# batra-mlp-lab/visdial

Measured on AMD Instinct MI355X. Metric: QA-rounds/sec training mn-att-ques-im-hist+disc (batch 20x10x100), higher is better.
Workload: dtype f32 operands and results; the option recurrence multiplies the EXACT 3-way bf16 split of both operands (9 bf16 MFMA products per fp32 product, f32 accumulate: fp32-grade, errors at the f32 MFMA's own level) -- its two step kernels and its weight-gradient contraction; f32 MFMA (v_mfma_f32_32x32x2_f32

## Files before the change

### visdial_amd/csrc/comm.hip

```cpp
#include <dlfcn.h>

#include "common.h"
#include "rt_core.h"
#include "../../include/visdial_hip.h"

namespace {

struct NcclUniqueId { char internal[128]; };
typedef void* NcclComm;
typedef int NcclResult;
enum { kNcclFloat32 = 7, kNcclSum = 0 };

struct Rccl {
  void* lib = nullptr;
  NcclResult (*GetUniqueId)(NcclUniqueId*) = nullptr;
  NcclResult (*CommInitRank)(NcclComm*, int, NcclUniqueId, int) = nullptr;
  NcclResult (*CommDestroy)(NcclComm) = nullptr;
  NcclResult (*AllReduce)(const void*, void*, size_t, int, int, NcclComm, hipStream_t) = nullptr;
  NcclResult (*GroupStart)() = nullptr;
  NcclResult (*GroupEnd)() = nullptr;
  const char* (*GetErrorString)(NcclResult) = nullptr;
  NcclResult (*GetVersion)(int*) = nullptr;
};

// ... 152 lines not shown
  if (g.stream) (void)hipStreamSynchronize(g.stream);
  NcclResult r = g.api.CommDestroy(g.comm);
  release_local();
  if (r != 0) {
    vd_set_error("vd_comm_destroy: ncclCommDestroy -> %s", g.api.GetErrorString(r));
    return VD_ERR_HIP;
  }
  return VD_OK;
}

int vd_model_allreduce_grads(vd_model* m) {
  VdRange r("vd_model_allreduce_grads");
  VD_CHECK_ARG(m, "vd_model_allreduce_grads: null model");
  VD_CHECK_ARG(g.comm, "vd_model_allreduce_grads: no communicator (vd_comm_init first)");
  VD_CHECK_ARG(m->cur >= 0, "vd_model_allreduce_grads: no backward pass has been enqueued");
  int dev = -1;
  VD_HIP(hipGetDevice(&dev));
  VD_CHECK_ARG(dev == g.device, "vd_model_allreduce_grads: communicator lives on device %d, current device is %d", g.device, dev);
  int64_t lo = 0, hi = 0;
  int rc = vd_model_encoder_range(m, &lo, &hi);
  if (rc != VD_OK) return rc;
  const bool split = hi > lo && m->enc_grads_recorded;
  if (split) {
    VD_HIP(hipStreamWaitEvent(g.stream, m->ev_enc_grads, 0));
    VD_NCCL(g.api.AllReduce(m->G + lo, m->G + lo, (size_t)(hi - lo), kNcclFloat32, kNcclSum, g.comm, g.stream));
    VD_HIP(hipEventRecord(g.ev_b1, g.stream));
    VD_HIP(hipEventRecord(g.ev_tail_t, m->s_main));
  }
  g.timed = split;
  VD_HIP(hipEventRecord(g.ev_tail, m->s_main));
// ... 26 lines not shown
```

### visdial_amd/csrc/rt_core.h

```cpp
#pragma once
#include <math.h>
#include <stdarg.h>
#include <stdlib.h>
#include <string.h>

#include <algorithm>
#include <map>
#include <memory>
#include <numeric>
#include <random>
#include <string>
#include <vector>

#include "../../include/visdial_hip.h"
#include "common.h"
#include "paths.h"

int vd_lstm2_forward_p(const vd_lstm2_fwd_t* st, int nstacks, int H, int flags, hipStream_t stream);
int vd_lstm2_backward_p(const vd_lstm2_bwd_t* st, int nstacks, int H, int flags, hipStream_t stream);

int vd_img_drop_gather(const float* pre, const uint8_t* mask1, float* xdrop, int N, int R, int S2, int H, float scale, hipStream_t stream);
int vd_img_common_forward_p(const float* pre, const uint8_t* mask1, const float* xdrop, const float* Wc, const float* bc, const float* qc,
                            const uint8_t* mask2, float* iqc, int N, int R, int S2, int H, int Kc, float scale, int flags, hipStream_t stream);
int vd_img_tr_backward_p(const float* dz, const float* Wc, const float* p, const float* datt, const uint8_t* mask1, float* dpre, int N, int R,
// ... 150 lines not shown
  vd_model_params p;
  int flags = 0;
  std::string enc_name, dec_name;
  std::vector<vdrt::Tensor> spec;
  std::map<std::string, int> index;
  long numel = 0;
  float *W = nullptr, *G = nullptr, *M = nullptr, *V = nullptr;
  std::map<std::string, vdrt::DevBuf> ws;
  std::map<std::string, vdrt::DevBuf> ext_masks;
  hipStream_t s_main = nullptr, s_side = nullptr;
  hipStream_t s_wg = nullptr;
  bool wg_active = false, wg_used = false;
  std::vector<hipEvent_t> ev_pool;
  size_t ev_next = 0;
  hipEvent_t ev_enc_grads = nullptr;
  hipEvent_t ev_updated = nullptr;
  bool updated_recorded = false;
  bool enc_grads_recorded = false;
  hipEvent_t ev_loss = nullptr, ev_prof[6] = {nullptr, nullptr, nullptr, nullptr, nullptr, nullptr};
  bool training = true, streams = true, prof_valid = false;
  long step = 0;
  int adam_t = 0;
  double lr = 1e-3;
  vdrt::BatchSlot slot[2];
  int cur = -1, uploaded = -1;
  float* loss_host = nullptr;
  long loss_cap = 0, loss_n = 0;
  bool loss_is_sum = false;
  std::unique_ptr<vdrt::Encoder> enc;
  std::unique_ptr<vdrt::Decoder> dec;
// ... 70 lines not shown
  VD_HIP(hipEventRecord(e, from));
  VD_HIP(hipStreamWaitEvent(side, e, 0));
  return VD_OK;
}
inline int join_stream(vd_model* m, hipStream_t side, hipStream_t to) { return fork_stream(m, side, to); }
inline hipStream_t side_stream(vd_model* m, hipStream_t cur) { return m->streams ? m->s_side : cur; }
inline int wg_fork(vd_model* m, hipStream_t cur, hipStream_t* out) {
  *out = cur;
  if (!m->wg_active || !m->s_wg) return VD_OK;
  VD_TRY(fork_stream(m, cur, m->s_wg));
  m->wg_used = true;
  *out = m->s_wg;
  return VD_OK;
}

inline int drop_mask(vd_model* m, const std::string& site, size_t numel, float p, hipStream_t s, uint8_t** out) {
  *out = nullptr;
  if (!m->training || p <= 0.f) return VD_OK;
  auto it = m->ext_masks.find(site);
  if (it != m->ext_masks.end()) {
    VD_CHECK_ARG(it->second.bytes >= numel, "dropout mask '%s' holds %zu bytes, the batch needs %zu", site.c_str(),
                 it->second.bytes, numel);
    *out = static_cast<uint8_t*>(it->second.p);
    return VD_OK;
  }
  if (!m->ext_masks.empty()) {
    vd_set_error("external dropout masks are set but none for site '%s'", site.c_str());
    return VD_ERR_STATE;
  }
  uint8_t* buf = nullptr;
// ... 46 lines not shown
    x = x_; M = M_; tanh_ = tanh;
    VD_TRY(ws_get(m, name + ".y", (size_t)M * out, &y));
    VD_TRY(vd_gemm_nt(x, in, Wp(m, name + ".W"), in, Wp(m, name + ".b"), y, out, (int)M, (int)out, (int)in,
                      tanh ? VD_ACT_TANH : VD_ACT_NONE, 0, s));
    if (y_out) *y_out = y;
    return VD_OK;
  }
  int backward(vd_model* m, hipStream_t s, const float* dy, bool need_dx, float** dx_out) {
    const float* d = dy;
    if (tanh_) {
      float* dpre;
      VD_TRY(ws_get(m, name + ".dpre", (size_t)M * out, &dpre));
      VD_TRY(vd_tanh_backward(dy, y, dpre, M * out, s));
      d = dpre;
    }
    VD_TRY(vd_gemm_tn_acc(d, out, x, in, Gp(m, name + ".W"), in, (int)out, (int)in, (int)M, 0, s));
    VD_TRY(vd_colsum_acc(d, out, (int)M, (int)out, Gp(m, name + ".b"), s));
    if (dx_out) *dx_out = nullptr;
    if (need_dx) {
      float* dx;
      VD_TRY(ws_get(m, name + ".dx", (size_t)M * in, &dx));
      VD_TRY(vd_gemm_nn(d, out, Wp(m, name + ".W"), in, nullptr, dx, in, (int)M, (int)in, (int)out, 0, s));
      if (dx_out) *dx_out = dx;
    }
    return VD_OK;
  }
};

struct CatLinear {
  std::string name;
  std::vector<long> dims;
  long D = 0, H = 0, N = 0;
// ... 122 lines not shown
      } else {
        VD_TRY(vd_gemm_nn(x, D, Wx(m), 4 * H, Wp(m, name + ".b"), gates, 4 * H, T * N, (int)(4 * H), (int)D, 0, s));
      }
      VD_TRY(vd_lstm_forward(gates, (int64_t)N * 4 * H, 4 * H, nullptr, mask, Wh(m), h0, c0, gates_out, h, c, T, N, (int)H, flags, s));
    }
    if (h_out) *h_out = h;
    return VD_OK;
  }
  int param_grads(vd_model* m, hipStream_t s, const std::vector<bool>& need_dx, std::vector<float*>* dxs) {
    const long TN = (long)T * N;
    float* dW = Gp(m, name + ".W");
    float* dWh = dW + D * 4 * H;
    const bool by_rows = rows && rows->act;
    auto dense_fits = [&](long Mrows, long K) { return vd_tn_kmajor_fits(Mrows, 4 * H, K); };
    auto wg_flags = [&](long Mrows) { return (m->flags & VD_FLAG_BF16) && vd_tn_split_tiles(Mrows, 4 * H) ? VD_FLAG_BF16 : 0; };
    if (by_rows && !(T > 1 && dense_fits(H, (long)(T - 1) * N))) {
      if (rows->n_act1 > 0)
        VD_TRY(vd_gemm_tn_rows_acc(h, H, rows->prev1, gates, 4 * H, rows->act1, dWh, 4 * H, (int)H, (int)(4 * H), rows->n_act1, s));
    } else if (T > 1) {
      VD_TRY(vd_gemm_tn_acc(h, H, gates + (long)N * 4 * H, 4 * H, dWh, 4 * H, (int)H, (int)(4 * H), (T - 1) * N, wg_flags(H), s));
    }
    if (h0) VD_TRY(vd_gemm_tn_acc(h0, H, gates, 4 * H, dWh, 4 * H, (int)H, (int)(4 * H), N, 0, s));
    VD_TRY(vd_colsum_acc(gates, 4 * H, (int)TN, (int)(4 * H), Gp(m, name + ".b"), s));
    if (dxs) dxs->assign(parts.size(), nullptr);
    long roff = 0;
    for (size_t i = 0; i < parts.size(); ++i) {
      if (by_rows && !dense_fits(parts[i], TN)) {
        if (rows->n_act > 0)
          VD_TRY(vd_gemm_tn_rows_acc(xs[i], parts[i], rows->act, gates, 4 * H, rows->act, dW + roff * 4 * H, 4 * H, (int)parts[i],
                                     (int)(4 * H), rows->n_act, s));
      } else {
        VD_TRY(vd_gemm_tn_acc(xs[i], parts[i], gates, 4 * H, dW + roff * 4 * H, 4 * H, (int)parts[i], (int)(4 * H), (int)TN, wg_flags(parts[i]), s));
      }
      if (need_dx.empty() || need_dx[i]) {
        float* dx;
        VD_TRY(ws_get(m, name + ".dx" + std::to_string(i), (size_t)TN * parts[i], &dx));
        VD_TRY(vd_gemm_nt(gates, 4 * H, Wx(m) + roff * 4 * H, 4 * H, nullptr, dx, parts[i], (int)TN, (int)parts[i], (int)(4 * H),
                          VD_ACT_NONE, 0, s));
        if (dxs) (*dxs)[i] = dx;
      }
      roff += parts[i];
    }
    return VD_OK;
  }
  int backward(vd_model* m, hipStream_t s, const float* dh_seq, const float* dh_last, const std::vector<bool>& need_dx,
               std::vector<float*>* dxs) {
    if (gradPrevOutput) {
// ... 42 lines not shown
```

### visdial_amd/csrc/rt_decoders.h

```cpp
#pragma once
#include "rt_encoders.h"

namespace vdrt {

int option_cache_resolve(vd_model* m, BatchSlot& sl, const int32_t* options, long NO, int To, hipStream_t s);

struct Decoder {
  virtual ~Decoder() {}
  virtual void declare(vd_model* m) = 0;
  virtual int forward_backward(vd_model* m, BatchSlot& b, bool only_forward) = 0;
  virtual int retrieve(vd_model* m, BatchSlot& b) = 0;
  virtual int retrieve_lhood(vd_model*, BatchSlot&) {
    vd_set_error("vd_model_retrieve_lhood: the live-row log-likelihood head scores candidates of decoder 'gen'; this model's decoder is 'disc'");
    return VD_ERR_ARG;
  }
  virtual int gen_begin(vd_model*, const int32_t*, int) { return no_gen(); }
  virtual int gen_step(vd_model*, const int32_t*, float*) { return no_gen(); }
  virtual int gen_select(vd_model*, const int32_t*, int) { return no_gen(); }
  virtual int gen_beam_search(vd_model*, int, int, int, int, int32_t*, double*) { return no_gen(); }
  virtual int gen_sample(vd_model*, int, int, int, double, const double*, int32_t*, double*) { return no_gen(); }
  static int no_gen() {
    vd_set_error("sampling / beam search only for the generative decoder (model.lua:436-438)");
    return VD_ERR_STATE;
  }
// ... 89 lines not shown
      VD_TRY(vd_memset(d_optH, 0, (long)NO * H * 4, s));
      VD_TRY(vd_embed_scatter_acc(d_optH, b.opt_uid, nullptr, d_optH_full, NOfull, (int)H, 1.f, s));
    }
    VD_TRY(stage_loss(m, loss_rows, N, false, s));
    m->scores = scores;
    m->prof_valid = !only_forward;
    if (only_forward) return VD_OK;
    VD_TRY(fork_stream(m, s, sd));
    float *dc, *dtab;
    int32_t* perm = b.opt_sort_perm;
    VD_TRY(ws_get(m, "opt.dc", (size_t)NO * H, &dc));
    VD_TRY(ws_get(m, "opt.dtable", (size_t)(V + 1) * 4 * H, &dtab));
    VD_CHECK_ARG(perm, "decoder 'disc': the batch slot carries no option-token sort");
    VD_TRY(vd_memset(dtab, 0, (V + 1) * 4 * H * 4, sd));
    VD_HIP(hipEventRecord(m->ev_prof[2], s));
    m->wg_active = m->streams && m->s_wg && (flags & VD_FLAG_BF16) != 0;
    m->wg_used = false;
    auto enc_bwd = [&]() -> int {
      VdRange r("encoder backward");
      VD_TRY(m->enc->backward(m, sd, b, d_enc));
      VD_PROBE_REC(1, sd);
      if (m->wg_used) VD_PROBE_REC(2, m->s_wg);
      if (m->wg_used) {
        VD_TRY(fork_stream(m, sd, m->s_wg));
        VD_HIP(hipEventRecord(m->ev_enc_grads, m->s_wg));
      } else {
        VD_HIP(hipEventRecord(m->ev_enc_grads, sd));
      }
      m->enc_grads_recorded = true;
      return VD_OK;
    };
    {
      VdRange r("disc: option LSTM backward");
      if (c16) VD_TRY(vd_lstm_backward_c16(Wopt + E * 4 * H, gates16, c, d_optH, dc, To, NO, (int)H, s));
      else VD_TRY(vd_lstm_backward(Wopt + E * 4 * H, gates, c, nullptr, nullptr, d_optH, nullptr, dc, nullptr, nullptr, nullptr, To, NO, (int)H, flags, s));
    }
    VD_HIP(hipEventRecord(m->ev_prof[3], s));
    VD_TRY(enc_bwd());
// ... 634 lines not shown
```

### visdial_amd/csrc/rt_encoders.h

```cpp
#pragma once
#include "rt_core.h"

namespace vdrt {

struct Encoder {
  virtual ~Encoder() {}
  virtual void declare(vd_model* m) = 0;
  virtual int forward(vd_model* m, hipStream_t s, BatchSlot& b, float** out) = 0;
  virtual int backward(vd_model* m, hipStream_t s, BatchSlot& b, const float* grad_out) = 0;
  virtual std::vector<SeqLSTM>* rnnLayers() { return nullptr; }
  virtual int seqLen(const BatchSlot& b) const { return b.q.T; }
};

inline int tick_flags(const vd_model* m) { return m->flags & VD_FLAG_BF16; }

inline int causal_mask(vd_model* m, int B, int R, uint8_t** out) {
  const std::string key = "causal." + std::to_string(B);
  DevBuf& d = m->ws[key];
  const size_t n = (size_t)B * R * R;
  if (!d.p) {
    std::vector<uint8_t> host(n);
    for (int r = 0; r < B * R; ++r)
      for (int j = 0; j < R; ++j) host[(size_t)r * R + j] = j > (r % R) ? 1 : 0;
    VD_HIP(hipMalloc(&d.p, n + 16));
// ... 288 lines not shown
    const float* dcur;
    VD_TRY(dropout_fwd(m, "att.du1", du1d, m_u, 2.f, (long)N * H, s, &dcur));
    float *dpre, *dscore;
    VD_TRY(ws_get(m, "att.dpre", (size_t)b.B * S2 * H, &dpre));
    VD_TRY(ws_get(m, "att.dscore", (size_t)N * S2, &dscore));
    VD_TRY(vd_memset(dpre, 0, (long)b.B * S2 * H * 4, s));
    for (int i = L - 1; i >= 0; --i) {
      const std::string sf = hop_sfx(i);
      float *dqc, *duq, *dun;
      VD_TRY(ws_get(m, "att.dqc" + sf, (size_t)N * K, &dqc));
      VD_TRY(ws_get(m, "att.du0" + sf, (size_t)N * H, &dun));
      VD_TRY(vd_img_att_backward(iqc[i], Wp(m, "att" + sf + ".W"), pre, m1, m2[i], patt[i], dcur, Gp(m, "att" + sf + ".W"),
                                 Gp(m, "att" + sf + ".b"), dqc, dscore, N, R, S2, (int)H, (int)K, sc, s));
      hipStream_t sw;
      VD_TRY(wg_fork(m, s, &sw));
      VD_TRY(vd_colsum_acc(iqc[i], K, N * S2, (int)K, Gp(m, "img_common" + sf + ".b"), sw));
      VD_TRY(vd_img_common_wgrad_p(iqc[i], pre, m1, xdrop, Gp(m, "img_common" + sf + ".W"), N, R, S2, (int)H, (int)K, sc, iflags, sw));
      VD_TRY(vd_img_tr_backward_p(iqc[i], Wp(m, "img_common" + sf + ".W"), patt[i], dcur, m1, dpre, N, R, S2, (int)H, (int)K, sc, iflags, sw));
      VD_TRY(ques_common[i].backward(m, s, dqc, true, &duq));
      VD_TRY(vd_axpby(duq, dcur, dun, (long)N * H, 1.f, 1.f, s));
      dcur = dun;
    }
    hipStream_t sw;
    VD_TRY(wg_fork(m, s, &sw));
    VD_TRY(img_proj.backward(m, sw, dpre, false, nullptr));
    *du0 = const_cast<float*>(dcur);
    return VD_OK;
  }
};

struct GraphEncoder : Encoder {
  bool memory_ = false, san_ = false, qi_ = false, qh_ = false;
  TextBranches text;
  MemoryBlock memory;
  SANBlock san;
  CatLinear qi, qh;
  explicit GraphEncoder(const std::string& name) {
    memory_ = name.rfind("mn", 0) == 0;
    san_ = name.find("att") != std::string::npos;
    qi_ = name == "mn-ques-im-hist";
// ... 347 lines not shown
```

### visdial_amd/csrc/runtime.hip

```cpp
#include <errno.h>
#include <float.h>

#include "rt_decoders.h"

using namespace vdrt;

vd_model::~vd_model() {}

namespace {

int upload_tokens(BatchSlot& sl, SeqTok& ss, const std::string& tag, const int32_t* rows_major, int N, int T, bool sorted, hipStream_t s) {
  ss.T = T;
  ss.N = N;
  ss.present = true;
  ss.sorted = sorted;
  const size_t TN = (size_t)T * N;
  const size_t total = sorted ? 7 * TN + 2 * (size_t)N + T : TN;
  int32_t* stage = nullptr;
  VD_TRY(pin_get(sl.pinned, tag + ".stage", total * sizeof(int32_t), (void**)&stage));
  int32_t* tok = stage;
  std::vector<int> len(sorted ? N : 0);
  for (int n = 0; n < N; ++n) {
    int first = T;
    for (int t = 0; t < T; ++t) {
// ... 203 lines not shown
  sl.tree_ok = false;
  const long V = m->p.vocabSize;
  for (size_t r = 0; r < (size_t)N * O; ++r) {
    bool run = true;
    for (int t = 0; t < T; ++t) {
      const int32_t a = oin[r * T + t], b = oout[r * T + t];
      if (a < 0 || a > V || b < 0 || b > V || (a != 0 && !run)) return VD_OK;
      run = run && a != 0;
    }
  }
  VD_TRY(tree_chunks(m, sl, oin, oout, N, O, T, 0, O, s));
  sl.tree_ok = true;
  return VD_OK;
}

extern "C" {

int vd_model_create(const vd_model_params* p, const char* encoder, const char* decoder, vd_model** out) {
  VD_CHECK_ARG(p && encoder && decoder && out, "vd_model_create: null argument");
  std::unique_ptr<Encoder> enc = make_encoder(encoder);
  std::unique_ptr<Decoder> dec = make_decoder(decoder);
  if (!enc || !dec) {
    vd_set_error("vd_model_create: unknown plug-in pair '%s' + '%s' (encoders: lf-ques, lf-ques-im, lf-ques-hist, lf-ques-im-hist, "
                 "lf-att-ques-im-hist, hre-ques-hist, hre-ques-im-hist, hrea-ques-im-hist, mn-ques-hist, mn-ques-im-hist, "
                 "mn-att-ques-im-hist; decoders: disc, gen)", encoder, decoder);
    return VD_ERR_ARG;
  }
  const std::string en(encoder);
  const bool use_im = has(en, "im"), is_att = has(en, "att") && !has(en, "hrea");
  VD_CHECK_ARG(p->rnnHiddenSize > 0 && p->rnnHiddenSize % 32 == 0 && p->embedSize > 0 && p->embedSize % 4 == 0 && p->vocabSize > 0 &&
// ... 98 lines not shown
  m->beam_no_repeat = beam_no_repeat;
  m->beam_length_penalty = beam_length_penalty;
  m->flags = flags;
  m->ocache.capacity = cache_rows;
  m->lhood_tree = lhood_tree;
  if (m->p.numAttentionLayers < 1 || has(en, "lf-att")) m->p.numAttentionLayers = 1;
  if (m->p.numLayers < 1) m->p.numLayers = 2;
  m->enc_name = encoder;
  m->dec_name = decoder;
  m->use_im = use_im;
  m->use_hist = has(en, "hist");
  m->is_att = is_att;
  m->is_graph = en.rfind("mn", 0) == 0 || en.rfind("lf-att", 0) == 0;
  m->lr = p->learningRate;
  m->streams = p->useStreams != 0;
  m->enc = std::move(enc);
  m->dec = std::move(dec);
  m->spec.push_back(Tensor{"embed", 0, p->vocabSize + 1, p->embedSize, 0});
  m->enc->declare(m);
  m->dec->declare(m);
  long off = 0;
  for (size_t i = 0; i < m->spec.size(); ++i) {
    m->spec[i].off = off;
    m->index[m->spec[i].name] = (int)i;
    off += (m->spec[i].numel() + 3) / 4 * 4;
  }
  m->numel = off;
  auto fail = [&](int rc) {
    vd_model_destroy(m);
    return rc;
// ... 18 lines not shown
  if (hipEventCreateWithFlags(&m->ev_loss, hipEventDisableTiming) != hipSuccess) return fail(VD_ERR_HIP);
  if (hipEventCreateWithFlags(&m->ev_enc_grads, hipEventDisableTiming) != hipSuccess) return fail(VD_ERR_HIP);
  if (hipEventCreateWithFlags(&m->ev_updated, hipEventDisableTiming) != hipSuccess) return fail(VD_ERR_HIP);
  for (auto& e : m->ev_prof)
    if (hipEventCreate(&e) != hipSuccess) return fail(VD_ERR_HIP);
  for (auto& sl : m->slot)
    if (hipEventCreateWithFlags(&sl.ready, hipEventDisableTiming) != hipSuccess ||
        hipEventCreateWithFlags(&sl.done, hipEventDisableTiming) != hipSuccess)
      return fail(VD_ERR_HIP);
  *out = m;
  return VD_OK;
}

void vd_model_destroy(vd_model* m) {
  if (!m) return;
  (void)hipDeviceSynchronize();
  for (float* v : {m->W, m->G, m->M, m->V})
    if (v) (void)hipFree(v);
  for (auto& kv : m->ws)
    if (kv.second.p) (void)hipFree(kv.second.p);
  for (auto& kv : m->ext_masks)
    if (kv.second.p) (void)hipFree(kv.second.p);
  if (m->ocache.table) (void)hipFree(m->ocache.table);
  for (auto& sl : m->slot) {
    for (auto& kv : sl.bufs)
      if (kv.second.p) (void)hipFree(kv.second.p);
    for (auto& kv : sl.pinned)
      if (kv.second.p) (void)hipHostFree(kv.second.p);
    if (sl.ready) (void)hipEventDestroy(sl.ready);
    if (sl.done) (void)hipEventDestroy(sl.done);
// ... 19 lines not shown
int vd_model_tensor_info(const vd_model* m, int64_t i, char* name64, int64_t* offset, int64_t* rows, int64_t* cols) {
  VD_CHECK_ARG(m && i >= 0 && i < (int64_t)m->spec.size(), "vd_model_tensor_info: bad index");
  const Tensor& t = m->spec[i];
  if (name64) {
    strncpy(name64, t.name.c_str(), 63);
    name64[63] = 0;
  }
  if (offset) *offset = t.off;
  if (rows) *rows = t.rows;
  if (cols) *cols = t.cols;
  return VD_OK;
}

int vd_model_flat_pointers(vd_model* m, float** W, float** dW, float** adam_m, float** adam_v) {
  VD_CHECK_ARG(m, "vd_model_flat_pointers: null model");
  m->ocache.flush();
  if (W) *W = m->W;
  if (dW) *dW = m->G;
  if (adam_m) *adam_m = m->M;
  if (adam_v) *adam_v = m->V;
  return VD_OK;
}

void* vd_model_stream(vd_model* m) { return m ? (void*)m->s_main : nullptr; }

int vd_model_encoder_range(const vd_model* m, int64_t* lo, int64_t* hi) {
  VD_CHECK_ARG(m && lo && hi, "vd_model_encoder_range: null");
  const char* first_dec = m->dec_name == "disc" ? "opt.W" : "dec1.W";
  *lo = m->spec[1].off;
  *hi = m->spec[m->index.at(first_dec)].off;
  return VD_OK;
}
int vd_model_wait_encoder_grads(vd_model* m, void* stream) {
  VD_CHECK_ARG(m && m->enc_grads_recorded, "vd_model_wait_encoder_grads: no backward pass has been enqueued");
  VD_HIP(hipStreamWaitEvent((hipStream_t)stream, m->ev_enc_grads, 0));
  return VD_OK;
}

int vd_model_init_params(vd_model* m, uint64_t seed) {
  VD_CHECK_ARG(m, "vd_model_init_params: null model");
  std::mt19937_64 rng(seed);
  std::vector<float> host((size_t)m->numel, 0.f);
  const long H = m->p.rnnHiddenSize;
  for (const Tensor& t : m->spec) {
    float* w = host.data() + t.off;
    const long n = t.numel();
    if (t.kind == 0) {
      std::normal_distribution<float> nd(0.f, 1.f);
      for (long i = t.cols; i < n; ++i) w[i] = nd(rng);
    } else if (t.kind == 1) {
      std::normal_distribution<float> nd(0.f, 1.f / sqrtf((float)t.rows));
      for (long i = 0; i < n; ++i) w[i] = nd(rng);
    } else if (t.kind == 2) {
      for (long i = H; i < 2 * H; ++i) w[i] = 1.f;
    } else {
      const long in = t.kind == 3 ? t.cols : m->spec[m->index.at(t.name.substr(0, t.name.size() - 2) + ".W")].cols;
      const float s = 1.f / sqrtf((float)in);
      std::uniform_real_distribution<float> ud(-s, s);
      for (long i = 0; i < n; ++i) w[i] = ud(rng);
    }
  }
  VD_HIP(hipMemcpy(m->W, host.data(), host.size() * sizeof(float), hipMemcpyHostToDevice));
  m->ocache.flush();
  return VD_OK;
}

int vd_model_set_tensor(vd_model* m, const char* name, const float* host, int64_t n) {
  VD_CHECK_ARG(m && name && host && m->index.count(name), "vd_model_set_tensor: unknown tensor '%s'", name ? name : "(null)");
  const Tensor& t = m->spec[m->index.at(name)];
  VD_CHECK_ARG(n == t.numel(), "vd_model_set_tensor: '%s' holds %ld values, got %ld", name, t.numel(), (long)n);
  VD_HIP(hipStreamSynchronize(m->s_main));
  VD_HIP(hipMemcpy(m->W + t.off, host, n * sizeof(float), hipMemcpyHostToDevice));
  m->ocache.flush();
  return VD_OK;
}

int vd_model_get_tensor(vd_model* m, const char* name, int which, float* host, int64_t n) {
  VD_CHECK_ARG(m && name && host && m->index.count(name), "vd_model_get_tensor: unknown tensor '%s'", name ? name : "(null)");
  const Tensor& t = m->spec[m->index.at(name)];
  VD_CHECK_ARG(n == t.numel() && which >= 0 && which <= 3, "vd_model_get_tensor: bad size / selector");
  VD_HIP(hipStreamSynchronize(m->s_main));
  float* base[4] = {m->W, m->G, m->M, m->V};
  VD_HIP(hipMemcpy(host, base[which] + t.off, n * sizeof(float), hipMemcpyDeviceToHost));
  return VD_OK;
}

int vd_model_set_training(vd_model* m, int on) {
  VD_CHECK_ARG(m, "vd_model_set_training: null model");
  m->training = on != 0;
  if (on) m->ocache.flush();
  return VD_OK;
}

int vd_model_set_dropout_mask(vd_model* m, const char* site, const uint8_t* host, int64_t n) {
  VD_CHECK_ARG(m, "vd_model_set_dropout_mask: null model");
  VD_HIP(hipStreamSynchronize(m->s_main));
  if (!host) {
    for (auto& kv : m->ext_masks)
      if (kv.second.p) VD_HIP(hipFree(kv.second.p));
    m->ext_masks.clear();
    return VD_OK;
  }
  VD_CHECK_ARG(site && n > 0, "vd_model_set_dropout_mask: bad arguments");
  void* p = nullptr;
  VD_TRY(dev_get(m->ext_masks, site, (size_t)n, &p));
  VD_HIP(hipMemcpy(p, host, (size_t)n, hipMemcpyHostToDevice));
  return VD_OK;
}

int vd_model_upload_batch(vd_model* m, const vd_batch* hb) {
// ... 95 lines not shown
  VD_TRY(pin_get(sl.pinned, "gt.stage", (size_t)N * sizeof(int32_t), (void**)&gp));
  for (int n = 0; n < N; ++n) {
    const int g = hb->answer_ind ? hb->answer_ind[n] - 1 : 0;
    VD_CHECK_ARG(!hb->answer_ind || (g >= 0 && g < O), "vd_model_upload_batch: answer_ind[%d] = %d out of 1..%d", n, g + 1, O);
    sl.gt_host[n] = g;
    gp[n] = g;
  }
  VD_TRY(dev_get(sl.bufs, "gt", (size_t)N * sizeof(int32_t), (void**)&sl.gt));
  VD_HIP(hipMemcpyAsync(sl.gt, gp, (size_t)N * sizeof(int32_t), hipMemcpyHostToDevice, s));
  VD_HIP(hipEventRecord(sl.ready, s));
  m->uploaded = (int)(&sl - m->slot);
  m->lhood_exec = -1;
  return VD_OK;
}

static int begin_step(vd_model* m, bool zero_grads, BatchSlot** out) {
  VD_CHECK_ARG(m && m->uploaded >= 0, "no batch uploaded");
  m->cur = m->uploaded;
  m->enc_grads_recorded = false;
  m->lhood_exec = -1;
  BatchSlot& b = m->slot[m->cur];
  m->N = b.q.N;
  m->O = m->p.numOptions;
  hipStream_t s = m->s_main;
  VD_HIP(hipStreamWaitEvent(s, b.ready, 0));
  if (zero_grads) VD_TRY(vd_memset(m->G, 0, m->numel * 4, s));
  VD_TRY(vd_memset(Wp(m, "embed"), 0, (long)m->p.embedSize * 4, s));
  b.used = true;
  *out = &b;
  return VD_OK;
}

int vd_model_forward_backward(vd_model* m, int only_forward) {
  VdRange r(only_forward ? "vd_model_forward" : "vd_model_forward_backward");
  BatchSlot* b = nullptr;
  VD_TRY(begin_step(m, !only_forward, &b));
  if (!only_forward) m->ocache.flush();
  const int rc = m->dec->forward_backward(m, *b, only_forward != 0);
  VD_HIP(hipEventRecord(b->done, m->s_main));
  return rc;
}

int vd_model_retrieve(vd_model* m) {
  VdRange r("vd_model_retrieve");
  BatchSlot* b = nullptr;
  VD_TRY(begin_step(m, false, &b));
  const int rc = m->dec->retrieve(m, *b);
  VD_HIP(hipEventRecord(b->done, m->s_main));
  return rc;
}

int vd_model_retrieve_lhood(vd_model* m) {
  VdRange r("vd_model_retrieve_lhood");
  BatchSlot* b = nullptr;
  VD_TRY(begin_step(m, false, &b));
  const int rc = m->dec->retrieve_lhood(m, *b);
  VD_HIP(hipEventRecord(b->done, m->s_main));
  return rc;
}

int vd_model_encode(vd_model* m) {
  BatchSlot* b = nullptr;
  VD_TRY(begin_step(m, false, &b));
  m->gen_enc_out = nullptr;
  float* out = nullptr;
  const int rc = m->enc->forward(m, m->s_main, *b, &out);
  VD_HIP(hipEventRecord(b->done, m->s_main));
  if (rc == VD_OK) {
    m->gen_enc_out = out;
    m->gen_seq_len = m->enc->seqLen(*b);
  }
  return rc;
}
int vd_model_decode_begin(vd_model* m, const int32_t* rounds, int n) {
  VD_CHECK_ARG(m, "vd_model_decode_begin: null model");
  return m->dec->gen_begin(m, rounds, n);
// ... 23 lines not shown
  VD_CHECK_ARG(m && loss && m->cur >= 0 && m->loss_n > 0, "vd_model_loss: nothing to read");
  VD_HIP(hipEventSynchronize(m->ev_loss));
  double s = 0;
  for (long i = 0; i < m->loss_n; ++i) s += m->loss_host[i];
  *loss = (float)(m->loss_is_sum ? s : s / (double)m->loss_n);
  return VD_OK;
}

int vd_model_update(vd_model* m, float gscale) {
  VD_CHECK_ARG(m, "vd_model_update: null model");
  VdRange r("vd_model_update: clamp + adam");
  m->adam_t += 1;
  m->ocache.flush();
  const double t = m->adam_t;
  const float step = (float)(m->lr * sqrt(1.0 - pow(0.999, t)) / (1.0 - pow(0.9, t)));
  VD_TRY(vd_clamp_adam(m->W, m->G, m->M, m->V, m->numel, gscale, 5.0f, 0.9f, 0.999f, 1e-8f, step, m->s_main));
  VD_HIP(hipEventRecord(m->ev_updated, m->s_main));
  m->updated_recorded = true;
  if (m->lr > m->p.minLRate) m->lr *= m->p.lrDecayRate;
  m->step += 1;
  return VD_OK;
}

int vd_model_learning_rate(vd_model* m, double* lr, int set) {
  VD_CHECK_ARG(m && lr, "vd_model_learning_rate: null");
  if (set) m->lr = *lr;
  else *lr = m->lr;
  return VD_OK;
}

// ... 44 lines not shown
int vd_model_option_rows(vd_model* m, int64_t* executed, int64_t* total) {
  VD_CHECK_ARG(m && executed && total && (m->cur >= 0 || m->uploaded >= 0), "vd_model_option_rows: no batch uploaded");
  if (m->lhood_exec >= 0) {
    *executed = m->lhood_exec;
    *total = m->lhood_total;
    return VD_OK;
  }
  const BatchSlot& b = m->slot[m->cur >= 0 ? m->cur : m->uploaded];
  *executed = b.opt.present ? b.opt.N : 0;
  *total = b.opt.present ? (b.opt_total ? b.opt_total : b.opt.N) : 0;
  return VD_OK;
}

int vd_model_synchronize(vd_model* m) {
  VD_CHECK_ARG(m, "vd_model_synchronize: null model");
  for (hipStream_t s : {m->s_side, m->s_wg, m->s_main})
    if (s) VD_HIP(hipStreamSynchronize(s));
  return VD_OK;
}

}
```

### visdial_amd/native.py

```python
import ctypes as C

import numpy as np

from . import _lib
from .split_eval import SplitEval

call = _lib.call


class _DevArray(object):

    def __init__(self, ptr, n):
        self.__cuda_array_interface__ = {'shape': (n,), 'typestr': '<f4', 'data': (ptr, False), 'version': 2}


class _Optims(object):

    def __init__(self, model):
        self._m = model

    def _lr(self, value=None):
        v = C.c_double(0.0 if value is None else float(value))
        call("vd_model_learning_rate", self._m.h, C.byref(v), 0 if value is None else 1)
        return float(v.value)
# ... 100 lines not shown
            a = np.empty(self._shape(name, r, c), np.float32)
            call("vd_model_get_tensor", self.h, name.encode(), which, a.ctypes.data, a.size)
            out[name] = a
        return out

    def get_parameters_dict(self):
        return self._get(0)

    def get_gradients_dict(self):
        return self._get(1)

    @property
    def wrapperW(self):
        if self._W is None:
            import torch
            ptrs = [C.c_void_p() for _ in range(4)]
            call("vd_model_flat_pointers", self.h, *[C.byref(x) for x in ptrs])
            n = int(_lib.load().vd_model_flat_size(self.h))
            self._W = torch.as_tensor(_DevArray(ptrs[0].value, n), device='cuda')
        self.synchronize()
        return self._W

    def _entries(self):
        kind = lambda n: 'embed' if n == 'embed' else ('lstm' if n.split('.')[0].rstrip('0123456789') in
                                                        ('hist', 'ques', 'opt', 'dec', 'dialog') else 'lin') + \
            ('_w' if n.endswith('.W') else '_b')
        return [(n, self._shape(n, r, c), kind(n)) for n, _, r, c in self.tensors]

    def load_flat_parameters(self, modelW):
        from . import t7
        self.set_parameters_dict(t7.flat_to_named(np.asarray(modelW), self._entries(), self.params['encoder']))

    def flat_parameters(self):
        from . import t7
# ... 204 lines not shown
```

Before: 8937.

## Defer encoder weight-gradient GEMMs and Adam update into next step's side stream

Encoder backward weight-gradient kernels (linear, LSTM, attention) are recorded as closures instead of being launched. They are replayed on the side stream at the start of the next forward_backward, together with the encoder-slice Adam update and gradient zeroing, so they overlap with the next step's forward. The decoder-side Adam runs immediately on the split ranges. Every API entry that observes parameters or gradients adds a flush to keep results consistent. The cost is extra bookkeeping, std::function overhead, and risk of ordering bugs around the encoder parameters the next forward reads before its deferred Adam update.

```diff
diff --git a/visdial_amd/csrc/comm.hip b/visdial_amd/csrc/comm.hip
--- a/visdial_amd/csrc/comm.hip
+++ b/visdial_amd/csrc/comm.hip
@@ -190,6 +190,7 @@
   VD_CHECK_ARG(m, "vd_model_allreduce_grads: null model");
   VD_CHECK_ARG(g.comm, "vd_model_allreduce_grads: no communicator (vd_comm_init first)");
   VD_CHECK_ARG(m->cur >= 0, "vd_model_allreduce_grads: no backward pass has been enqueued");
+  VD_TRY(vdrt::defer_flush(m, true));
   int dev = -1;
   VD_HIP(hipGetDevice(&dev));
   VD_CHECK_ARG(dev == g.device, "vd_model_allreduce_grads: communicator lives on device %d, current device is %d", g.device, dev);
diff --git a/visdial_amd/csrc/rt_core.h b/visdial_amd/csrc/rt_core.h
--- a/visdial_amd/csrc/rt_core.h
+++ b/visdial_amd/csrc/rt_core.h
@@ -5,6 +5,7 @@
 #include <string.h>
 
 #include <algorithm>
+#include <functional>
 #include <map>
 #include <memory>
 #include <numeric>
@@ -188,6 +189,9 @@
   std::vector<hipEvent_t> ev_pool;
   size_t ev_next = 0;
   hipEvent_t ev_enc_grads = nullptr;
+  bool defer_on = false, defer_rec = false, defer_adam = false;
+  std::vector<std::function<int(hipStream_t)>> defer_list;
+  float defer_gscale = 1.f, defer_step = 0.f;
   hipEvent_t ev_updated = nullptr;
   bool updated_recorded = false;
   bool enc_grads_recorded = false;
@@ -288,6 +292,18 @@
   return VD_OK;
 }
 
+template <class F>
+inline int wg_launch(vd_model* m, hipStream_t s, F&& f) {
+  if (!m->defer_rec) return f(s);
+  m->defer_list.emplace_back(std::forward<F>(f));
+  return VD_OK;
+}
+int defer_run(vd_model* m, bool join, bool zero);
+inline int defer_flush(vd_model* m, bool disable = false) {
+  if (disable) m->defer_on = false;
+  return defer_run(m, true, false);
+}
+
 inline int drop_mask(vd_model* m, const std::string& site, size_t numel, float p, hipStream_t s, uint8_t** out) {
   *out = nullptr;
   if (!m->training || p <= 0.f) return VD_OK;
@@ -364,8 +380,15 @@
       VD_TRY(vd_tanh_backward(dy, y, dpre, M * out, s));
       d = dpre;
     }
-    VD_TRY(vd_gemm_tn_acc(d, out, x, in, Gp(m, name + ".W"), in, (int)out, (int)in, (int)M, 0, s));
-    VD_TRY(vd_colsum_acc(d, out, (int)M, (int)out, Gp(m, name + ".b"), s));
+    {
+      const float* x_ = x;
+      float *dWt = Gp(m, name + ".W"), *db = Gp(m, name + ".b");
+      const long in_ = in, out_ = out, M_ = M;
+      VD_TRY(wg_launch(m, s, [=](hipStream_t sw) -> int {
+        VD_TRY(vd_gemm_tn_acc(d, out_, x_, in_, dWt, in_, (int)out_, (int)in_, (int)M_, 0, sw));
+        return vd_colsum_acc(d, out_, (int)M_, (int)out_, db, sw);
+      }));
+    }
     if (dx_out) *dx_out = nullptr;
     if (need_dx) {
       float* dx;
@@ -518,23 +541,47 @@
     const bool by_rows = rows && rows->act;
     auto dense_fits = [&](long Mrows, long K) { return vd_tn_kmajor_fits(Mrows, 4 * H, K); };
     auto wg_flags = [&](long Mrows) { return (m->flags & VD_FLAG_BF16) && vd_tn_split_tiles(Mrows, 4 * H) ? VD_FLAG_BF16 : 0; };
+    const float *h_ = h, *g_ = gates, *h0_ = h0;
+    const long H_ = H;
+    const int T_ = T, N_ = N;
+    float* db = Gp(m, name + ".b");
     if (by_rows && !(T > 1 && dense_fits(H, (long)(T - 1) * N))) {
-      if (rows->n_act1 > 0)
-        VD_TRY(vd_gemm_tn_rows_acc(h, H, rows->prev1, gates, 4 * H, rows->act1, dWh, 4 * H, (int)H, (int)(4 * H), rows->n_act1, s));
+      if (rows->n_act1 > 0) {
+        const int32_t *prev1 = rows->prev1, *act1 = rows->act1;
+        const int n1 = rows->n_act1;
+        VD_TRY(wg_launch(m, s, [=](hipStream_t sw) -> int {
+          return vd_gemm_tn_rows_acc(h_, H_, prev1, g_, 4 * H_, act1, dWh, 4 * H_, (int)H_, (int)(4 * H_), n1, sw);
+        }));
+      }
     } else if (T > 1) {
-      VD_TRY(vd_gemm_tn_acc(h, H, gates + (long)N * 4 * H, 4 * H, dWh, 4 * H, (int)H, (int)(4 * H), (T - 1) * N, wg_flags(H), s));
-    }
-    if (h0) VD_TRY(vd_gemm_tn_acc(h0, H, gates, 4 * H, dWh, 4 * H, (int)H, (int)(4 * H), N, 0, s));
-    VD_TRY(vd_colsum_acc(gates, 4 * H, (int)TN, (int)(4 * H), Gp(m, name + ".b"), s));
+      const int fl = wg_flags(H);
+      VD_TRY(wg_launch(m, s, [=](hipStream_t sw) -> int {
+        return vd_gemm_tn_acc(h_, H_, g_ + (long)N_ * 4 * H_, 4 * H_, dWh, 4 * H_, (int)H_, (int)(4 * H_), (T_ - 1) * N_, fl, sw);
+      }));
+    }
+    VD_TRY(wg_launch(m, s, [=](hipStream_t sw) -> int {
+      if (h0_) VD_TRY(vd_gemm_tn_acc(h0_, H_, g_, 4 * H_, dWh, 4 * H_, (int)H_, (int)(4 * H_), N_, 0, sw));
+      return vd_colsum_acc(g_, 4 * H_, (int)TN, (int)(4 * H_), db, sw);
+    }));
     if (dxs) dxs->assign(parts.size(), nullptr);
     long roff = 0;
     for (size_t i = 0; i < parts.size(); ++i) {
+      const float* x_ = xs[i];
+      const long Pi = parts[i];
+      float* dWi = dW + roff * 4 * H;
       if (by_rows && !dense_fits(parts[i], TN)) {
-        if (rows->n_act > 0)
-          VD_TRY(vd_gemm_tn_rows_acc(xs[i], parts[i], rows->act, gates, 4 * H, rows->act, dW + roff * 4 * H, 4 * H, (int)parts[i],
-                                     (int)(4 * H), rows->n_act, s));
+        if (rows->n_act > 0) {
+          const int32_t* act = rows->act;
+          const int na = rows->n_act;
+          VD_TRY(wg_launch(m, s, [=](hipStream_t sw) -> int {
+            return vd_gemm_tn_rows_acc(x_, Pi, act, g_, 4 * H_, act, dWi, 4 * H_, (int)Pi, (int)(4 * H_), na, sw);
+          }));
+        }
       } else {
-        VD_TRY(vd_gemm_tn_acc(xs[i], parts[i], gates, 4 * H, dW + roff * 4 * H, 4 * H, (int)parts[i], (int)(4 * H), (int)TN, wg_flags(parts[i]), s));
+        const int fl = wg_flags(parts[i]);
+        VD_TRY(wg_launch(m, s, [=](hipStream_t sw) -> int {
+          return vd_gemm_tn_acc(x_, Pi, g_, 4 * H_, dWi, 4 * H_, (int)Pi, (int)(4 * H_), (int)TN, fl, sw);
+        }));
       }
       if (need_dx.empty() || need_dx[i]) {
         float* dx;
diff --git a/visdial_amd/csrc/rt_decoders.h b/visdial_amd/csrc/rt_decoders.h
--- a/visdial_amd/csrc/rt_decoders.h
+++ b/visdial_amd/csrc/rt_decoders.h
@@ -127,14 +127,19 @@
     VD_CHECK_ARG(perm, "decoder 'disc': the batch slot carries no option-token sort");
     VD_TRY(vd_memset(dtab, 0, (V + 1) * 4 * H * 4, sd));
     VD_HIP(hipEventRecord(m->ev_prof[2], s));
-    m->wg_active = m->streams && m->s_wg && (flags & VD_FLAG_BF16) != 0;
+    m->wg_active = !m->defer_on && m->streams && m->s_wg && (flags & VD_FLAG_BF16) != 0;
     m->wg_used = false;
     auto enc_bwd = [&]() -> int {
       VdRange r("encoder backward");
-      VD_TRY(m->enc->backward(m, sd, b, d_enc));
+      m->defer_rec = m->defer_on;
+      const int rc = m->enc->backward(m, sd, b, d_enc);
+      m->defer_rec = false;
+      if (rc != VD_OK) m->defer_list.clear();
+      VD_TRY(rc);
       VD_PROBE_REC(1, sd);
       if (m->wg_used) VD_PROBE_REC(2, m->s_wg);
-      if (m->wg_used) {
+      if (!m->defer_list.empty()) {
+      } else if (m->wg_used) {
         VD_TRY(fork_stream(m, sd, m->s_wg));
         VD_HIP(hipEventRecord(m->ev_enc_grads, m->s_wg));
       } else {
diff --git a/visdial_amd/csrc/rt_encoders.h b/visdial_amd/csrc/rt_encoders.h
--- a/visdial_amd/csrc/rt_encoders.h
+++ b/visdial_amd/csrc/rt_encoders.h
@@ -326,16 +326,25 @@
                                  Gp(m, "att" + sf + ".b"), dqc, dscore, N, R, S2, (int)H, (int)K, sc, s));
       hipStream_t sw;
       VD_TRY(wg_fork(m, s, &sw));
-      VD_TRY(vd_colsum_acc(iqc[i], K, N * S2, (int)K, Gp(m, "img_common" + sf + ".b"), sw));
-      VD_TRY(vd_img_common_wgrad_p(iqc[i], pre, m1, xdrop, Gp(m, "img_common" + sf + ".W"), N, R, S2, (int)H, (int)K, sc, iflags, sw));
-      VD_TRY(vd_img_tr_backward_p(iqc[i], Wp(m, "img_common" + sf + ".W"), patt[i], dcur, m1, dpre, N, R, S2, (int)H, (int)K, sc, iflags, sw));
+      {
+        const float *dz = iqc[i], *pre_ = pre, *xd = xdrop, *p_ = patt[i], *Wc = Wp(m, "img_common" + sf + ".W");
+        const uint8_t* mk = m1;
+        float *dWc = Gp(m, "img_common" + sf + ".W"), *dbc = Gp(m, "img_common" + sf + ".b");
+        const int N_ = N, R_ = R, S2_ = S2, H_ = (int)H, K_ = (int)K, fl = iflags;
+        const float sc_ = sc;
+        VD_TRY(wg_launch(m, sw, [=](hipStream_t st) -> int {
+          VD_TRY(vd_colsum_acc(dz, K_, N_ * S2_, K_, dbc, st));
+          VD_TRY(vd_img_common_wgrad_p(dz, pre_, mk, xd, dWc, N_, R_, S2_, H_, K_, sc_, fl, st));
+          return vd_img_tr_backward_p(dz, Wc, p_, dcur, mk, dpre, N_, R_, S2_, H_, K_, sc_, fl, st);
+        }));
+      }
       VD_TRY(ques_common[i].backward(m, s, dqc, true, &duq));
       VD_TRY(vd_axpby(duq, dcur, dun, (long)N * H, 1.f, 1.f, s));
       dcur = dun;
     }
     hipStream_t sw;
     VD_TRY(wg_fork(m, s, &sw));
-    VD_TRY(img_proj.backward(m, sw, dpre, false, nullptr));
+    VD_TRY(wg_launch(m, sw, [this, m, dpre](hipStream_t st) -> int { return img_proj.backward(m, st, dpre, false, nullptr); }));
     *du0 = const_cast<float*>(dcur);
     return VD_OK;
   }
diff --git a/visdial_amd/csrc/runtime.hip b/visdial_amd/csrc/runtime.hip
--- a/visdial_amd/csrc/runtime.hip
+++ b/visdial_amd/csrc/runtime.hip
@@ -241,6 +241,29 @@
   return VD_OK;
 }
 
+int vdrt::defer_run(vd_model* m, bool join, bool zero) {
+  if (m->defer_list.empty() && !m->defer_adam) return VD_OK;
+  VdRange r("deferred encoder parameter gradients");
+  hipStream_t s = m->s_main, sd = m->s_side;
+  std::vector<std::function<int(hipStream_t)>> list;
+  list.swap(m->defer_list);
+  const bool adam = m->defer_adam;
+  m->defer_adam = false;
+#ifdef VD_PROBE_SKIP_ENC_WG
+  list.clear();
+#endif
+  int64_t lo = 0, hi = 0;
+  VD_TRY(vd_model_encoder_range(m, &lo, &hi));
+  VD_TRY(fork_stream(m, s, sd));
+  for (auto& f : list) VD_TRY(f(sd));
+  if (!list.empty()) VD_HIP(hipEventRecord(m->ev_enc_grads, sd));
+  if (adam)
+    VD_TRY(vd_clamp_adam(m->W + lo, m->G + lo, m->M + lo, m->V + lo, hi - lo, m->defer_gscale, 5.0f, 0.9f, 0.999f, 1e-8f, m->defer_step, sd));
+  if (zero) VD_TRY(vd_memset(m->G + lo, 0, (hi - lo) * 4, sd));
+  if (join) VD_TRY(join_stream(m, sd, s));
+  return VD_OK;
+}
+
 extern "C" {
 
 int vd_model_create(const vd_model_params* p, const char* encoder, const char* decoder, vd_model** out) {
@@ -369,6 +392,13 @@
   m->is_graph = en.rfind("mn", 0) == 0 || en.rfind("lf-att", 0) == 0;
   m->lr = p->learningRate;
   m->streams = p->useStreams != 0;
+  {
+    bool on = true;
+    if (const char* e = getenv("VD_DEFER_ENC_WG")) on = atol(e) != 0;
+    int world = 0;
+    (void)vd_comm_info(nullptr, &world);
+    m->defer_on = on && m->dec_name == "disc" && m->streams && world == 0;
+  }
   m->enc = std::move(enc);
   m->dec = std::move(dec);
   m->spec.push_back(Tensor{"embed", 0, p->vocabSize + 1, p->embedSize, 0});
@@ -417,6 +447,7 @@
 
 void vd_model_destroy(vd_model* m) {
   if (!m) return;
+  (void)vdrt::defer_flush(m);
   (void)hipDeviceSynchronize();
   for (float* v : {m->W, m->G, m->M, m->V})
     if (v) (void)hipFree(v);
@@ -466,6 +497,7 @@
 
 int vd_model_flat_pointers(vd_model* m, float** W, float** dW, float** adam_m, float** adam_v) {
   VD_CHECK_ARG(m, "vd_model_flat_pointers: null model");
+  VD_TRY(defer_flush(m, dW != nullptr));
   m->ocache.flush();
   if (W) *W = m->W;
   if (dW) *dW = m->G;
@@ -485,12 +517,15 @@
 }
 int vd_model_wait_encoder_grads(vd_model* m, void* stream) {
   VD_CHECK_ARG(m && m->enc_grads_recorded, "vd_model_wait_encoder_grads: no backward pass has been enqueued");
+  VD_TRY(defer_flush(m, true));
   VD_HIP(hipStreamWaitEvent((hipStream_t)stream, m->ev_enc_grads, 0));
   return VD_OK;
 }
 
 int vd_model_init_params(vd_model* m, uint64_t seed) {
   VD_CHECK_ARG(m, "vd_model_init_params: null model");
+  VD_TRY(defer_flush(m));
+  VD_HIP(hipStreamSynchronize(m->s_main));
   std::mt19937_64 rng(seed);
   std::vector<float> host((size_t)m->numel, 0.f);
   const long H = m->p.rnnHiddenSize;
@@ -521,6 +556,7 @@
   VD_CHECK_ARG(m && name && host && m->index.count(name), "vd_model_set_tensor: unknown tensor '%s'", name ? name : "(null)");
   const Tensor& t = m->spec[m->index.at(name)];
   VD_CHECK_ARG(n == t.numel(), "vd_model_set_tensor: '%s' holds %ld values, got %ld", name, t.numel(), (long)n);
+  VD_TRY(defer_flush(m));
   VD_HIP(hipStreamSynchronize(m->s_main));
   VD_HIP(hipMemcpy(m->W + t.off, host, n * sizeof(float), hipMemcpyHostToDevice));
   m->ocache.flush();
@@ -531,6 +567,7 @@
   VD_CHECK_ARG(m && name && host && m->index.count(name), "vd_model_get_tensor: unknown tensor '%s'", name ? name : "(null)");
   const Tensor& t = m->spec[m->index.at(name)];
   VD_CHECK_ARG(n == t.numel() && which >= 0 && which <= 3, "vd_model_get_tensor: bad size / selector");
+  VD_TRY(defer_flush(m));
   VD_HIP(hipStreamSynchronize(m->s_main));
   float* base[4] = {m->W, m->G, m->M, m->V};
   VD_HIP(hipMemcpy(host, base[which] + t.off, n * sizeof(float), hipMemcpyDeviceToHost));
@@ -539,6 +576,7 @@
 
 int vd_model_set_training(vd_model* m, int on) {
   VD_CHECK_ARG(m, "vd_model_set_training: null model");
+  VD_TRY(defer_flush(m));
   m->training = on != 0;
   if (on) m->ocache.flush();
   return VD_OK;
@@ -546,6 +584,7 @@
 
 int vd_model_set_dropout_mask(vd_model* m, const char* site, const uint8_t* host, int64_t n) {
   VD_CHECK_ARG(m, "vd_model_set_dropout_mask: null model");
+  VD_TRY(defer_flush(m));
   VD_HIP(hipStreamSynchronize(m->s_main));
   if (!host) {
     for (auto& kv : m->ext_masks)
@@ -671,7 +710,7 @@
   return VD_OK;
 }
 
-static int begin_step(vd_model* m, bool zero_grads, BatchSlot** out) {
+static int begin_step(vd_model* m, bool zero_grads, BatchSlot** out, bool enc_zeroed = false) {
   VD_CHECK_ARG(m && m->uploaded >= 0, "no batch uploaded");
   m->cur = m->uploaded;
   m->enc_grads_recorded = false;
@@ -681,7 +720,14 @@
   m->O = m->p.numOptions;
   hipStream_t s = m->s_main;
   VD_HIP(hipStreamWaitEvent(s, b.ready, 0));
-  if (zero_grads) VD_TRY(vd_memset(m->G, 0, m->numel * 4, s));
+  if (zero_grads && enc_zeroed) {
+    int64_t lo = 0, hi = 0;
+    VD_TRY(vd_model_encoder_range(m, &lo, &hi));
+    VD_TRY(vd_memset(m->G, 0, lo * 4, s));
+    VD_TRY(vd_memset(m->G + hi, 0, (m->numel - hi) * 4, s));
+  } else if (zero_grads) {
+    VD_TRY(vd_memset(m->G, 0, m->numel * 4, s));
+  }
   VD_TRY(vd_memset(Wp(m, "embed"), 0, (long)m->p.embedSize * 4, s));
   b.used = true;
   *out = &b;
@@ -690,8 +736,17 @@
 
 int vd_model_forward_backward(vd_model* m, int only_forward) {
   VdRange r(only_forward ? "vd_model_forward" : "vd_model_forward_backward");
+  VD_CHECK_ARG(m && m->uploaded >= 0, "no batch uploaded");
+#ifdef VD_PROBE_EARLY_ENC_WG
+  const bool pending = false;
+  if (!only_forward) VD_TRY(defer_run(m, false, false));
+#else
+  const bool pending = !only_forward && (!m->defer_list.empty() || m->defer_adam);
+#endif
+  if (pending) VD_TRY(defer_run(m, false, true));
+  else VD_TRY(defer_flush(m));
   BatchSlot* b = nullptr;
-  VD_TRY(begin_step(m, !only_forward, &b));
+  VD_TRY(begin_step(m, !only_forward, &b, pending));
   if (!only_forward) m->ocache.flush();
   const int rc = m->dec->forward_backward(m, *b, only_forward != 0);
   VD_HIP(hipEventRecord(b->done, m->s_main));
@@ -700,6 +755,8 @@
 
 int vd_model_retrieve(vd_model* m) {
   VdRange r("vd_model_retrieve");
+  VD_CHECK_ARG(m, "vd_model_retrieve: null model");
+  VD_TRY(defer_flush(m));
   BatchSlot* b = nullptr;
   VD_TRY(begin_step(m, false, &b));
   const int rc = m->dec->retrieve(m, *b);
@@ -709,6 +766,8 @@
 
 int vd_model_retrieve_lhood(vd_model* m) {
   VdRange r("vd_model_retrieve_lhood");
+  VD_CHECK_ARG(m, "vd_model_retrieve_lhood: null model");
+  VD_TRY(defer_flush(m));
   BatchSlot* b = nullptr;
   VD_TRY(begin_step(m, false, &b));
   const int rc = m->dec->retrieve_lhood(m, *b);
@@ -717,6 +776,8 @@
 }
 
 int vd_model_encode(vd_model* m) {
+  VD_CHECK_ARG(m, "vd_model_encode: null model");
+  VD_TRY(defer_flush(m));
   BatchSlot* b = nullptr;
   VD_TRY(begin_step(m, false, &b));
   m->gen_enc_out = nullptr;
@@ -770,6 +831,18 @@
   m->ocache.flush();
   const double t = m->adam_t;
   const float step = (float)(m->lr * sqrt(1.0 - pow(0.999, t)) / (1.0 - pow(0.9, t)));
+  if (m->defer_adam) VD_TRY(defer_flush(m));
+#ifndef VD_PROBE_EARLY_ENC_WG
+  if (!m->defer_list.empty()) {
+    int64_t lo = 0, hi = 0;
+    VD_TRY(vd_model_encoder_range(m, &lo, &hi));
+    VD_TRY(vd_clamp_adam(m->W, m->G, m->M, m->V, lo, gscale, 5.0f, 0.9f, 0.999f, 1e-8f, step, m->s_main));
+    VD_TRY(vd_clamp_adam(m->W + hi, m->G + hi, m->M + hi, m->V + hi, m->numel - hi, gscale, 5.0f, 0.9f, 0.999f, 1e-8f, step, m->s_main));
+    m->defer_adam = true;
+    m->defer_gscale = gscale;
+    m->defer_step = step;
+  } else
+#endif
   VD_TRY(vd_clamp_adam(m->W, m->G, m->M, m->V, m->numel, gscale, 5.0f, 0.9f, 0.999f, 1e-8f, step, m->s_main));
   VD_HIP(hipEventRecord(m->ev_updated, m->s_main));
   m->updated_recorded = true;
@@ -844,6 +917,7 @@
 
 int vd_model_synchronize(vd_model* m) {
   VD_CHECK_ARG(m, "vd_model_synchronize: null model");
+  VD_TRY(defer_flush(m));
   for (hipStream_t s : {m->s_side, m->s_wg, m->s_main})
     if (s) VD_HIP(hipStreamSynchronize(s));
   return VD_OK;
diff --git a/visdial_amd/native.py b/visdial_amd/native.py
--- a/visdial_amd/native.py
+++ b/visdial_amd/native.py
@@ -138,10 +138,10 @@
     def wrapperW(self):
         if self._W is None:
             import torch
-            ptrs = [C.c_void_p() for _ in range(4)]
-            call("vd_model_flat_pointers", self.h, *[C.byref(x) for x in ptrs])
+            w = C.c_void_p()
+            call("vd_model_flat_pointers", self.h, C.byref(w), None, None, None)
             n = int(_lib.load().vd_model_flat_size(self.h))
-            self._W = torch.as_tensor(_DevArray(ptrs[0].value, n), device='cuda')
+            self._W = torch.as_tensor(_DevArray(w.value, n), device='cuda')
         self.synchronize()
         return self._W
 
```

After: 8898. About the same (-0.4%).
